# hpcaitech/SkyComputing

Measured on AMD Instinct MI355X. Metric: sec_per_iter_bert160_mnli_bsz32, lower is better.
Workload: dtype bf16; 1 GPU; model=bert-160L-H1024-A16, global_batch=32, seq_len=128, parallelism=pp1, microbatches=1, schedule=gpipe, allocate=even, num_pipeline_layers=483, hipgraph=True

## Files before the change

### skycomputing_amd/models/bert_layers.py

```python

from __future__ import annotations

import torch
import torch.nn as nn

from .. import ops
from ..registry import LAYER
from .bert import BertConfig


def _cfg(config) -> BertConfig:
    if isinstance(config, BertConfig):
        return config
    if isinstance(config, dict):
        return BertConfig.from_dict(config)
    raise TypeError(f"expected BertConfig or dict, got {type(config)}")


class SkyLayerNorm(nn.Module):

    def __init__(self, hidden_size: int, eps: float = 1e-12):
        super().__init__()
        self.weight = nn.Parameter(torch.ones(hidden_size))
        self.bias = nn.Parameter(torch.zeros(hidden_size))
# ... 107 lines not shown
    def activation_numel(self, batch: int, seq: int) -> int:
        return batch * seq * self.config.hidden_size + batch * seq


@LAYER.register_module(name="BertLayer_Head")
class BertLayerHead(nn.Module):

    def __init__(self, config):
        super().__init__()
        config = _cfg(config)
        self.config = config
        self.attention = BertSelfAttention(config)
        self.output = BertSelfOutput(config)

    def forward(self, hidden, ext_mask):
        attn = self.attention(hidden, ext_mask)
        out = self.output(attn, hidden)
        return out, ext_mask

    def layer_flops(self, batch: int, seq: int) -> float:
        H = self.config.hidden_size
        gemm = 4 * 2.0 * batch * seq * H * H
        attn = 2 * 2.0 * batch * self.config.num_attention_heads * seq * seq * (
            H // self.config.num_attention_heads
        )
        return gemm + attn

    def activation_numel(self, batch: int, seq: int) -> int:
        H = self.config.hidden_size
        h = self.config.num_attention_heads
        return 6 * batch * seq * H + 2 * batch * h * seq * seq

    def param_count(self) -> int:
# ... 106 lines not shown
```

### skycomputing_amd/ops/__init__.py

```python

from __future__ import annotations

import math
import os

import torch

from . import eager, hiplib
from .eager import ACT_FNS, gelu, swish

__all__ = [
    "layer_norm", "bias_gelu", "bias_tanh", "masked_softmax", "dropout",
    "attention_context", "linear_act", "linear_residual_layer_norm",
    "embedding_fused", "sgd_step",
    "gelu", "swish", "ACT_FNS", "hip_available",
]


def hip_available() -> bool:
    return hiplib.available()


def _use_hip(t: torch.Tensor) -> bool:
    if not t.is_cuda:
        return False
    if hiplib.available():
        return True
    if os.environ.get("SKY_ALLOW_EAGER_GPU") == "1":
# ... 107 lines not shown
        and _use_hip(x)
    ):
        from .functions import (
            LinearResidualLayerNormFn, ln_dbias_enabled, ln_xsum_width_ok,
        )

        if ln_dbias_enabled() and ln_xsum_width_ok(weight.shape[0]):
            p = dropout_p if training else 0.0
            return LinearResidualLayerNormFn.apply(
                x, weight, bias, ln_weight, ln_bias, eps, residual, p
            )
    return layer_norm(linear(x, weight, bias), ln_weight, ln_bias, eps,
                      residual, dropout_p, training)


def linear_act(x, weight, bias, act: str = "gelu"):
    if _use_hip(x) and act == "gelu" and bias is not None:
        from .functions import LinearGeluFn, _use_hblt

        if (_use_hblt() and os.environ.get("SKY_HBLT_GELU") == "1"
                and x.dtype == torch.float32 and weight.shape[0] % 8 == 0):
            return LinearGeluFn.apply(x, weight, bias)
        if x.dtype == torch.bfloat16:
            from .functions import _g2_enabled, _g2_fit

            rows = x.numel() // x.shape[-1]
            if (_g2_enabled("fwd", rows, weight.shape[0], weight.shape[1])
                    and _g2_fit(rows, weight.shape[0], weight.shape[1])):
                return LinearGeluFn.apply(x, weight, bias)
        y = torch.nn.functional.linear(x, weight)
# ... 25 lines not shown
```

### skycomputing_amd/ops/functions.py

```python

from __future__ import annotations

import os

import torch

from . import hiplib
from .hiplib import check, ptr

_DT = {torch.float32: 0, torch.bfloat16: 1}

_seed_gen = torch.Generator()
_seed_gen.manual_seed(0x5EED)


def set_dropout_seed(seed: int):
    _seed_gen.manual_seed(seed)


def _next_seed() -> int:
    return int(torch.randint(0, 2**62, (1,), generator=_seed_gen).item())


def _stream() -> int:
# ... 231 lines not shown
        "sky_masked_softmax_bwd",
    )
    dQ = torch.matmul(dS, k)
    dK = torch.matmul(dS.transpose(-1, -2), q)
    dqkv = torch.empty_like(qkv)
    check(
        lib.sky_pack3(
            _stream(), ptr(dQ.contiguous()), ptr(dK.contiguous()),
            ptr(dV.contiguous()), ptr(dqkv), B, S, h, d, _dt(qkv),
        ),
        "sky_pack3",
    )
    return dqkv


class FusedAttentionFn(torch.autograd.Function):

    @staticmethod
    def forward(ctx, qkv, mask, scale, dropout_p, training):
        lib = hiplib.require()
        B, S, three, h, d = qkv.shape
        assert three == 3 and d == 64 and S <= 128
        qkv = qkv.contiguous()
        mask = mask.contiguous() if mask is not None else None
        out = torch.empty(B, S, h, d, dtype=qkv.dtype, device=qkv.device)
        m = torch.empty(B, h, S, dtype=torch.float32, device=qkv.device)
        lsum = torch.empty_like(m)
        keep = 1.0 - dropout_p if (dropout_p > 0 and training) else 1.0
        salt = _next_seed() if keep < 1.0 else 0
        state = rng_state()
        check(
            lib.sky_attn_fwd(
                _stream(), ptr(qkv), ptr(mask), ptr(out), ptr(m), ptr(lsum),
                B, S, h, d, scale, keep, salt, state.data_ptr(),
            ),
            "sky_attn_fwd",
        )
        ctx.save_for_backward(qkv, mask, m, lsum)
        ctx.scale, ctx.keep, ctx.salt = scale, keep, salt
        return out

    @staticmethod
    def backward(ctx, dout):
        lib = hiplib.require()
        qkv, mask, m, lsum = ctx.saved_tensors
        B, S, _, h, d = qkv.shape
        dev = qkv.device
        if os.environ.get("SKY_NO_FUSED_ATTN_BWD") != "1":
            dout = dout.contiguous()
            dqkv = torch.empty_like(qkv)
            if os.environ.get("SKY_ATTN_FUSED_BWD") == "1":
                check(
                    lib.sky_attn_bwd_fused(
                        _stream(), ptr(qkv), ptr(dout), ptr(mask), ptr(m),
                        ptr(lsum), ptr(dqkv), B, S, h, d, ctx.scale,
                        ctx.keep, ctx.salt, rng_state().data_ptr(),
                    ),
                    "sky_attn_bwd_fused",
                )
                return dqkv, None, None, None, None
            alloc = torch.empty if S == 128 else torch.zeros
            n = B * h * S * S + (32 if S % 32 else 0)
            pdT = alloc(n, dtype=qkv.dtype, device=dev)
            dsT = alloc(n, dtype=qkv.dtype, device=dev)
            check(
                lib.sky_attn_bwd(
                    _stream(), ptr(qkv), ptr(dout), ptr(mask), ptr(m),
                    ptr(lsum), ptr(pdT), ptr(dsT), ptr(dqkv),
                    B, S, h, d, ctx.scale, ctx.keep, ctx.salt,
                    rng_state().data_ptr(),
                ),
                "sky_attn_bwd",
            )
            return dqkv, None, None, None, None
        P = torch.empty(B, h, S, S, dtype=qkv.dtype, device=dev)
        Pd = torch.empty_like(P) if ctx.keep < 1.0 else P
        check(
            lib.sky_attn_probs(
                _stream(), ptr(qkv), ptr(mask), ptr(m), ptr(lsum), ptr(P),
# ... 219 lines not shown


def gemm2_wgrad(dy2, x2):
    if dy2.dtype != torch.bfloat16:
        return None
    Kred, M = dy2.shape
    N = x2.shape[1]
    if not (_g2_enabled("wgrad", M, N, Kred) and _g2_fit(M, N, Kred)):
        return None
    dw = torch.empty(M, N, dtype=dy2.dtype, device=dy2.device)
    _g2_call(dy2, x2, dw, None, None, M, N, Kred, dy2.stride(0),
             x2.stride(0), dw.stride(0), 1, 1, 0, _g2_gsu(M, N, Kred))
    return dw


class LinearBiasFn(torch.autograd.Function):

    @staticmethod
    def forward(ctx, x, weight, bias):
        xs = x.shape
        x2 = x.reshape(-1, xs[-1])
        g2 = gemm2_fwd(x2 if x2.is_contiguous() else x2.contiguous(),
                       weight, bias)
        if g2 is not None:
            y = g2[0]
        else:
            y = torch.nn.functional.linear(x2, weight, bias)
        ctx.save_for_backward(x2, weight)
        ctx.xshape = xs
        ctx.has_bias = bias is not None
        return y.view(*xs[:-1], weight.shape[0])

    @staticmethod
    def backward(ctx, dy):
        x2, weight = ctx.saved_tensors
        dy2 = dy.reshape(-1, weight.shape[0])
        if not dy2.is_contiguous():
            dy2 = dy2.contiguous()
        dx = gemm2_dgrad(dy2, weight)
        dx = dx.view(ctx.xshape) if dx is not None else dy2.mm(weight).view(ctx.xshape)
        dw2 = gemm2_wgrad(dy2, x2 if x2.is_contiguous() else x2.contiguous())
        if dw2 is not None:
# ... 13 lines not shown
            )
            return dx, dw, db
        dw = dy2.t().mm(x2)
        db = colsum(dy2, weight.dtype) if ctx.has_bias else None
        return dx, dw, db


def ln_dbias_enabled() -> bool:
    return os.environ.get("SKY_NO_LN_DBIAS") != "1"


def ln_xsum_width_ok(cols: int) -> bool:
    return bool(hiplib.require().sky_layernorm_bwd_xsum_ok(cols))


class LinearResidualLayerNormFn(torch.autograd.Function):

    @staticmethod
    def forward(ctx, x, weight, bias, ln_w, ln_b, eps, residual, dropout_p=0.0):
        lib = hiplib.require()
        xs = x.shape
        x2 = x.reshape(-1, xs[-1])
        g2 = gemm2_fwd(x2 if x2.is_contiguous() else x2.contiguous(),
                       weight, bias)
        if g2 is not None:
            h = g2[0]
        else:
            h = torch.nn.functional.linear(x2, weight, bias)
        cols = weight.shape[0]
        h = h.view(*xs[:-1], cols).contiguous()
        residual = residual.contiguous() if residual is not None else None
        rows = h.numel() // cols
        y = torch.empty_like(h)
        mean = torch.empty(rows, dtype=torch.float32, device=h.device)
        rstd = torch.empty(rows, dtype=torch.float32, device=h.device)
        keep = 1.0 - dropout_p
        salt = _next_seed() if keep < 1.0 else 0
        state_ptr = rng_state().data_ptr() if keep < 1.0 else 0
        check(
            lib.sky_layernorm_fwd(
                _stream(), ptr(h), ptr(residual), ptr(ln_w), ptr(ln_b),
                ptr(y), ptr(mean), ptr(rstd), rows, cols, eps, _dt(h),
                keep, salt, state_ptr,
            ),
            "sky_layernorm_fwd",
        )
        ctx.save_for_backward(x2, weight, h, ln_w, mean, rstd)
        ctx.residual = residual
        ctx.has_residual = residual is not None
        ctx.keep, ctx.salt = keep, salt
        ctx.xshape = xs
        return y

    @staticmethod
    def backward(ctx, dy):
        lib = hiplib.require()
        x2, weight, h, ln_w, mean, rstd = ctx.saved_tensors
        dy = dy.contiguous()
        cols = h.shape[-1]
        rows = h.numel() // cols
        dh = torch.empty_like(h)
        d_ln_w = torch.empty(cols, dtype=ln_w.dtype, device=h.device)
        d_ln_b = torch.empty(cols, dtype=ln_w.dtype, device=h.device)
        dbias = torch.empty(cols, dtype=ln_w.dtype, device=h.device)
        scratch = _red_scratch(cols, 3, h.device)
        drop = ctx.keep < 1.0
        dres = torch.empty_like(h) if (drop and ctx.has_residual) else None
        state_ptr = rng_state().data_ptr() if drop else 0
        check(
            lib.sky_layernorm_bwd_xsum(
                _stream(), ptr(dy), ptr(h), ptr(ctx.residual), ptr(ln_w),
                ptr(mean), ptr(rstd), ptr(dh), ptr(d_ln_w), ptr(d_ln_b),
                ptr(scratch), rows, cols, _dt(h), ctx.keep, ctx.salt,
                state_ptr, ptr(dres), ptr(dbias),
            ),
            "sky_layernorm_bwd_xsum",
        )
        if not ctx.has_residual:
            dgrad_res = None
        elif drop:
            dgrad_res = dres
        else:
            dgrad_res = dh
        if dbias.dtype != weight.dtype:
            dbias = dbias.to(weight.dtype)
        dh2 = dh.view(-1, cols)
        dx = gemm2_dgrad(dh2, weight)
        dx = dx.view(ctx.xshape) if dx is not None else dh2.mm(weight).view(ctx.xshape)
        xc = x2 if x2.is_contiguous() else x2.contiguous()
        dw = gemm2_wgrad(dh2, xc)
        if dw is None and _use_hblt():
            M, K = xc.shape
            dw = torch.empty_like(weight)
            check(
                lib.sky_hblt_wgrad(
                    _stream(), ptr(xc), ptr(dh2), ptr(dw), M, cols, K, _dt(xc)
                ),
                "sky_hblt_wgrad",
            )
        elif dw is None:
            dw = dh2.t().mm(x2)
        return dx, dw, dbias, d_ln_w, d_ln_b, None, dgrad_res, None


class LinearGeluFn(torch.autograd.Function):

    @staticmethod
    def forward(ctx, x, weight, bias):
        xs = x.shape
        x2 = x.reshape(-1, xs[-1]).contiguous()
        M, K = x2.shape
        N = weight.shape[0]
        g2 = gemm2_fwd(x2, weight, bias, gelu=True, want_z=True)
        if g2 is not None:
            y, aux = g2
        else:
            lib = hiplib.require()
# ... 98 lines not shown
```

### skycomputing_amd/ops/hip/attention_bwd.hip

```cpp

#include "attn_common.h"

template <bool HAS_MASK>
__global__ __launch_bounds__(256, 3) void attn_bwd1s_kernel(
    const ushort_t* __restrict__ qkv, const ushort_t* __restrict__ dout,
    const ushort_t* __restrict__ mask, const float* __restrict__ m_io,
    const float* __restrict__ l_io, ushort_t* __restrict__ pdT,
    ushort_t* __restrict__ dsT, ushort_t* __restrict__ dqkv, int B, int S,
    int h, float scale, float keep, uint64_t salt,
    const unsigned long long* __restrict__ state) {
  extern __shared__ __attribute__((aligned(16))) char lds[];
  const int tid = threadIdx.x;
  const int l = tid & 63;
  const int w = tid >> 6;
  const int lm = l & 15;
  const int lg = l >> 4;
  const int QB = (S + 63) / 64;
  const int bh = blockIdx.x / QB;
  const int qb = blockIdx.x % QB;
  const int b = bh / h;
  const int hh = bh % h;
  const int ts = 3 * h * ATT_D;
  const int NT = (S + 15) / 16;
  const uint64_t seed = rng_seed(salt, state);
  const float inv_keep = 1.f / keep;
// ... 99 lines not shown
          *(ushort4_t*)(dsT + o) = ds4;
          *(ushort4_t*)(pdT + o) = pd4;
        } else {
#pragma unroll
          for (int r = 0; r < 4; ++r)
            if (qtok_base + lg * 4 + r < S) {
              dsT[o + r] = ds4[r];
              pdT[o + r] = pd4[r];
            }
        }
      }
    }
  }
  __syncthreads();

  if (active) {
    f32x4 qacc[4];
    att_zero(qacc);
#pragma unroll
    for (int ks = 0; ks < 4; ++ks) {
      if (ks * 32 >= S) break;
      bf16x8 asr = *(const bf16x8*)lds_at(
          lds, swz(32768 + w * 4096 + lm * 256 + (ks * 32 + lg * 8) * 2, lm, 15));
#pragma unroll
      for (int ct = 0; ct < 4; ++ct) {
        bf16x8 bkt = abf_tr_rows64(lds, 16384, ks * 32 + lg * 8, ct * 4, lm);
        qacc[ct] = __builtin_amdgcn_mfma_f32_16x16x32_bf16(asr, bkt, qacc[ct], 0, 0, 0);
      }
    }
    ushort_t* dq = dqkv + (size_t)b * S * ts + (size_t)hh * ATT_D;
    att_store_rows16(dq, ts, qacc, qtok_base, S, lm, lg);
  }
}

__global__ __launch_bounds__(256) void attn_bwd2_kernel(
    const ushort_t* __restrict__ qkv, const ushort_t* __restrict__ dout,
    const ushort_t* __restrict__ pdT, const ushort_t* __restrict__ dsT,
    ushort_t* __restrict__ dqkv, int B, int S, int h) {
  extern __shared__ __attribute__((aligned(16))) char lds[];
  const int tid = threadIdx.x;
  const int l = tid & 63;
  const int w = tid >> 6;
  const int lm = l & 15;
  const int lg = l >> 4;
  const int bh = blockIdx.x;
  const int b = bh / h;
  const int hh = bh % h;
  const int ts = 3 * h * ATT_D;
  const int dots = h * ATT_D;

  const ushort_t* qbase = qkv + (size_t)b * S * ts + (size_t)hh * ATT_D;
  const ushort_t* dobase = dout + ((size_t)b * S * h + hh) * ATT_D;

  att_glds_rows(qbase, ts, 0, S, false, S, lds, 0, tid);
  att_glds_rows(dobase, dots, 0, S, false, S, lds, 16384, tid);
  for (int u = S * 8 + tid; u < 128 * 8; u += 256) {
    *(ushort8_t*)lds_at(lds, 0 + u * 16) = (ushort8_t)(ushort_t)0;
    *(ushort8_t*)lds_at(lds, 16384 + u * 16) = (ushort8_t)(ushort_t)0;
  }
  asm volatile("s_waitcnt vmcnt(0)" ::: "memory");
  __syncthreads();

  const int kt0 = 2 * w;
  for (int ki = 0; ki < 2; ++ki) {
    const int ktok_base = (kt0 + ki) * 16;
    if (ktok_base >= S) break;
    int ktok = ktok_base + lm;
    if (ktok >= S) ktok = S - 1;
    f32x4 vacc[4], kacc[4];
    att_zero(vacc);
    att_zero(kacc);
#pragma unroll
    for (int ks = 0; ks < 4; ++ks) {
      if (ks * 32 >= S) break;
      const size_t abase = ((size_t)bh * S + ktok) * S + ks * 32 + lg * 8;
      bf16x8 apd = *(const bf16x8*)(pdT + abase);
      bf16x8 ads = *(const bf16x8*)(dsT + abase);
#pragma unroll
      for (int ct = 0; ct < 4; ++ct) {
        bf16x8 bdo = abf_tr_rows64(lds, 16384, ks * 32 + lg * 8, ct * 4, lm);
        vacc[ct] = __builtin_amdgcn_mfma_f32_16x16x32_bf16(apd, bdo, vacc[ct], 0, 0, 0);
        bf16x8 bq = abf_tr_rows64(lds, 0, ks * 32 + lg * 8, ct * 4, lm);
        kacc[ct] = __builtin_amdgcn_mfma_f32_16x16x32_bf16(ads, bq, kacc[ct], 0, 0, 0);
      }
    }
    ushort_t* dk = dqkv + (size_t)b * S * ts + (size_t)(h + hh) * ATT_D;
    ushort_t* dv = dqkv + (size_t)b * S * ts + (size_t)(2 * h + hh) * ATT_D;
    att_store_rows16x2(dk, dv, ts, kacc, vacc, ktok_base, S, lm, lg);
  }
}

#define ABF_K 0
#define ABF_Q (16 * 1024)
#define ABF_DO (32 * 1024)
#define ABF_DS (48 * 1024)
#define ABF_PD (64 * 1024)
#define ABF_LDS (80 * 1024)

template <bool HAS_MASK>
__global__ __launch_bounds__(256, 1) void attn_bwd_fused_kernel(
    const ushort_t* __restrict__ qkv, const ushort_t* __restrict__ dout,
    const ushort_t* __restrict__ mask, const float* __restrict__ m_io,
    const float* __restrict__ l_io, ushort_t* __restrict__ dqkv, int B,
// ... 177 lines not shown
                                  int64_t S, int64_t h, int64_t d,
                                  float scale, float keep, uint64_t salt,
                                  uint64_t state) {
  if (d != ATT_D || S > ATT_SMAX) return (int)hipErrorInvalidValue;
  hipStream_t s = (hipStream_t)stream;
  dim3 grid((unsigned)(B * h));
  ATT_LAUNCH_HM(mask != 0, (attn_bwd_fused_kernel<HM>), grid, ABF_LDS, s,
                (const ushort_t*)qkv, (const ushort_t*)dout,
                (const ushort_t*)mask, (const float*)m, (const float*)lsum,
                (ushort_t*)dqkv, (int)B, (int)S, (int)h, scale, keep, salt,
                (const unsigned long long*)state);
  LAUNCH_CHECK();
  return 0;
}

SKY_EXPORT int sky_attn_bwd(uint64_t stream, uint64_t qkv, uint64_t dout,
                            uint64_t mask, uint64_t m, uint64_t lsum,
                            uint64_t pdT, uint64_t dsT, uint64_t dqkv,
                            int64_t B, int64_t S, int64_t h, int64_t d,
                            float scale, float keep, uint64_t salt,
                            uint64_t state) {
  if (d != ATT_D || S > ATT_SMAX) return (int)hipErrorInvalidValue;
  hipStream_t s = (hipStream_t)stream;
  dim3 grid((unsigned)(B * h * ((S + 63) / 64)));
  ATT_LAUNCH_HM(mask != 0, (attn_bwd1s_kernel<HM>), grid, 48 * 1024, s,
                (const ushort_t*)qkv, (const ushort_t*)dout,
                (const ushort_t*)mask, (const float*)m, (const float*)lsum,
                (ushort_t*)pdT, (ushort_t*)dsT, (ushort_t*)dqkv, (int)B,
                (int)S, (int)h, scale, keep, salt,
                (const unsigned long long*)state);
  hipLaunchKernelGGL(attn_bwd2_kernel, dim3((unsigned)(B * h)), dim3(256),
                     32 * 1024, s, (const ushort_t*)qkv,
                     (const ushort_t*)dout, (const ushort_t*)pdT,
                     (const ushort_t*)dsT, (ushort_t*)dqkv, (int)B, (int)S,
                     (int)h);
  LAUNCH_CHECK();
  return 0;
}
```

### skycomputing_amd/ops/hip/attn_common.h

```cpp
#pragma once

#include "common.h"

typedef const __attribute__((address_space(1))) unsigned int* att_gas;
typedef __attribute__((address_space(3))) unsigned int* att_las;

typedef __attribute__((ext_vector_type(8))) short bf16x8;
typedef __attribute__((ext_vector_type(4))) float f32x4;

#define ATT_SMAX 128
#define ATT_D 64

DEV void* lds_at(char* base, int byte) { return (void*)(base + byte); }

DEV int swz(int byte_addr, int row, int rmask) {
  return byte_addr ^ ((row & rmask) << 4);
}

typedef __attribute__((ext_vector_type(4))) short s16x4_a;
typedef __attribute__((address_space(3))) s16x4_a* abf_las4;

DEV bf16x8 abf_tr_rows64(const char* lds_base, int off, int r0, int cq0,
                         int s4) {
  s16x4_a v[2];
// ... 121 lines not shown
                            int row0, int S, int lm, int lg) {
#pragma unroll
  for (int ct = 0; ct < 4; ++ct) {
#pragma unroll
    for (int r = 0; r < 4; ++r) {
      const int row = row0 + lg * 4 + r;
      const int c = ct * 16 + lm;
      if (row < S) {
        d0[(size_t)row * rstride + c] = f32_to_bf16(a0[ct][r]);
        d1[(size_t)row * rstride + c] = f32_to_bf16(a1[ct][r]);
      }
    }
  }
}

#define ATT_LAUNCH_HM(has_mask, KERNEL, grid, lds_bytes, stream, ...)         \
  do {                                                                        \
    if (has_mask) {                                                           \
      constexpr bool HM = true;                                               \
      hipLaunchKernelGGL(KERNEL, grid, dim3(256), lds_bytes, stream,          \
                         __VA_ARGS__);                                        \
    } else {                                                                  \
      constexpr bool HM = false;                                              \
      hipLaunchKernelGGL(KERNEL, grid, dim3(256), lds_bytes, stream,          \
                         __VA_ARGS__);                                        \
    }                                                                         \
  } while (0)
```

### skycomputing_amd/ops/hip/common.h

```cpp
#pragma once

#include <hip/hip_runtime.h>
#include <hip/hip_bf16.h>
#include <stdint.h>

#define WAVE 64
#define DEV __device__ __forceinline__

typedef unsigned short ushort_t;
typedef __attribute__((ext_vector_type(2))) unsigned short ushort2_t;
typedef __attribute__((ext_vector_type(4))) unsigned short ushort4_t;
typedef __attribute__((ext_vector_type(8))) unsigned short ushort8_t;
typedef __attribute__((ext_vector_type(4))) float float4_t;

DEV float bf16_to_f32(ushort_t u) {
  union { unsigned int i; float f; } v;
  v.i = ((unsigned int)u) << 16;
  return v.f;
}

DEV ushort_t f32_to_bf16(float f) {
  union { unsigned int i; float f; } v;
  v.f = f;
  unsigned int lsb = (v.i >> 16) & 1u;
// ... 108 lines not shown
  const float p = t * fmaf(t, fmaf(t, fmaf(t, fmaf(t, 1.061405429f, -1.453152027f),
                                           1.421413741f), -0.284496736f),
                           0.254829592f);
  const float r = 1.f - p * __expf(-ax * ax);
  return copysignf(r, x);
}
DEV float gelu_f(float x) { return 0.5f * x * (1.f + erf_fast(x * 0.70710678118654752f)); }
DEV float gelu_grad_f(float x) {
  const float k = 0.70710678118654752f;
  const float c = 0.3989422804014327f;
  float cdf = 0.5f * (1.f + erf_fast(x * k));
  float pdf = c * __expf(-0.5f * x * x);
  return cdf + x * pdf;
}

#define LAUNCH_CHECK() do { hipError_t e_ = hipGetLastError(); if (e_ != hipSuccess) return (int)e_; } while (0)

#define SKY_EXPORT extern "C" __attribute__((visibility("default")))
```

### skycomputing_amd/ops/hip/elementwise.hip

```cpp

#include "common.h"


template <int DT>
__global__ __launch_bounds__(256) void bias_gelu_fwd_vec_kernel(
    const void* __restrict__ x, const void* __restrict__ b,
    void* __restrict__ y, int64_t n8, int64_t cols8) {
  for (int64_t i8 = (int64_t)blockIdx.x * 256 + threadIdx.x; i8 < n8;
       i8 += (int64_t)gridDim.x * 256) {
    float v[8], bv[8];
    Vec8<DT>::load(x, i8, v);
    Vec8<DT>::load(b, i8 % cols8, bv);
#pragma unroll
    for (int j = 0; j < 8; ++j) v[j] = gelu_f(v[j] + bv[j]);
    Vec8<DT>::store(y, i8, v);
  }
}

template <int DT>
__global__ __launch_bounds__(256) void bias_gelu_fwd_kernel(
    const void* __restrict__ x, const void* __restrict__ b,
    void* __restrict__ y, int64_t n, int64_t cols) {
  for (int64_t i = (int64_t)blockIdx.x * 256 + threadIdx.x; i < n;
       i += (int64_t)gridDim.x * 256) {
// ... 153 lines not shown
  float s = 0.f;
  if (col < cols) {
    const int64_t y1 = min(nslabs, (int64_t)(g + 1) * per);
    for (int64_t y = (int64_t)g * per; y < y1; ++y)
      s += scratch[y * cols + col];
  }
  lds[g][c] = s;
  __syncthreads();
  for (int st = 32; st >= 1; st >>= 1) {
    if (g < st) lds[g][c] += lds[g + st][c];
    __syncthreads();
  }
  if (g == 0 && col < cols) store_elem<DTOUT>(out, col, lds[0][c]);
}

template <int DT, int BLOCK>
__global__ __launch_bounds__(BLOCK) void colsum_kernel(
    const void* __restrict__ src, float* __restrict__ out, int64_t rows,
    int64_t cols, int64_t rows_per_slab) {
  const int64_t col = (int64_t)blockIdx.x * BLOCK + threadIdx.x;
  if (col >= cols) return;
  const int64_t r0 = (int64_t)blockIdx.y * rows_per_slab;
  const int64_t r1 = min(rows, r0 + rows_per_slab);
  float s = 0.f;
  for (int64_t r = r0; r < r1; ++r) s += load_elem<DT>(src, r * cols + col);
  atomicAdd(&out[col], s);
}

template <int DT>
static void launch_colsum(hipStream_t s, const void* src, void* out,
                          float* scratch, int64_t rows, int64_t cols,
                          int dtout) {
  if (cols % 8 == 0 && scratch != nullptr) {
    constexpr int BLOCK = 128;
    const int64_t cols8 = cols / 8;
    const int64_t gx = (cols8 + BLOCK - 1) / BLOCK;
    int64_t nslabs = 1024 / gx;
    if (nslabs < 128) nslabs = 128;
    if (nslabs > CS_SLABS) nslabs = CS_SLABS;
    if (nslabs > rows) nslabs = rows;
    const int64_t slab = (rows + nslabs - 1) / nslabs;
    dim3 grid((unsigned)gx, (unsigned)nslabs);
    hipLaunchKernelGGL((colsum_part_kernel<DT, BLOCK>), grid, dim3(BLOCK), 0,
                       s, src, scratch, rows, cols8, slab);
    dim3 g2((unsigned)((cols + 15) / 16));
    if (dtout == DT_BF16)
      hipLaunchKernelGGL((colsum_final_kernel<256, DT_BF16>), g2, dim3(1024), 0,
                         s, scratch, out, cols, nslabs);
    else
      hipLaunchKernelGGL((colsum_final_kernel<256, DT_F32>), g2, dim3(1024), 0,
                         s, scratch, out, cols, nslabs);
    return;
  }
  constexpr int BLOCK = 256;
  int64_t slab = 64;
  while ((cols + BLOCK - 1) / BLOCK * ((rows + slab - 1) / slab) > 2048 && slab < rows)
    slab *= 2;
  dim3 grid((unsigned)((cols + BLOCK - 1) / BLOCK),
            (unsigned)((rows + slab - 1) / slab));
  (void)dtout;
  hipLaunchKernelGGL((colsum_kernel<DT, BLOCK>), grid, dim3(BLOCK), 0, s, src,
                     (float*)out, rows, cols, slab);
}

SKY_EXPORT int sky_colsum(uint64_t stream, uint64_t src, uint64_t out,
                          uint64_t scratch, int64_t rows, int64_t cols,
// ... 22 lines not shown
    if (nslabs > CS_SLABS) nslabs = CS_SLABS;
    if (nslabs > rows) nslabs = rows;
    const int64_t slab = (rows + nslabs - 1) / nslabs;
    dim3 grid((unsigned)(nwin * nslabs));
    auto launch_cs = [&](auto kern) {
      hipLaunchKernelGGL(kern, grid, dim3(256), 0, s, (const void*)dy,
                         (const void*)x, (const void*)b, (void*)dx,
                         (float*)scratch, rows, cols8, slab);
    };
    if (dt == DT_F32)
      hb ? launch_cs(bias_gelu_bwd_cs_kernel<DT_F32, true>)
         : launch_cs(bias_gelu_bwd_cs_kernel<DT_F32, false>);
    else
      hb ? launch_cs(bias_gelu_bwd_cs_kernel<DT_BF16, true>)
         : launch_cs(bias_gelu_bwd_cs_kernel<DT_BF16, false>);
    dim3 g2((unsigned)((cols + 15) / 16));
    if (dt == DT_BF16)
      hipLaunchKernelGGL((colsum_final_kernel<256, DT_BF16>), g2, dim3(1024),
                         0, s, (float*)scratch, (void*)db, cols, nslabs);
    else
      hipLaunchKernelGGL((colsum_final_kernel<256, DT_F32>), g2, dim3(1024),
                         0, s, (float*)scratch, (void*)db, cols, nslabs);
    LAUNCH_CHECK();
    return 0;
  }
  if (cols % 8 == 0 && scratch != 0 && getenv("SKY_GELU_FUSED_BWD")) {
    constexpr int BLOCK = 128;
    const int64_t cols8 = cols / 8;
    const int64_t gx = (cols8 + BLOCK - 1) / BLOCK;
    int64_t nslabs = 4096 / gx;
    if (nslabs < 128) nslabs = 128;
    if (nslabs > CS_SLABS) nslabs = CS_SLABS;
    if (nslabs > rows) nslabs = rows;
    const int64_t slab = (rows + nslabs - 1) / nslabs;
    dim3 grid((unsigned)gx, (unsigned)nslabs);
    auto launch_part = [&](auto kern) {
      hipLaunchKernelGGL(kern, grid, dim3(BLOCK), 0, s, (const void*)dy,
                         (const void*)x, (const void*)b, (void*)dx,
                         (float*)scratch, rows, cols8, slab);
    };
    if (dt == DT_F32)
      hb ? launch_part(bias_gelu_bwd_part_kernel<DT_F32, true, BLOCK>)
         : launch_part(bias_gelu_bwd_part_kernel<DT_F32, false, BLOCK>);
    else
      hb ? launch_part(bias_gelu_bwd_part_kernel<DT_BF16, true, BLOCK>)
         : launch_part(bias_gelu_bwd_part_kernel<DT_BF16, false, BLOCK>);
    dim3 g2((unsigned)((cols + 15) / 16));
    if (dt == DT_BF16)
      hipLaunchKernelGGL((colsum_final_kernel<256, DT_BF16>), g2, dim3(1024),
                         0, s, (float*)scratch, (void*)db, cols, nslabs);
    else
      hipLaunchKernelGGL((colsum_final_kernel<256, DT_F32>), g2, dim3(1024),
                         0, s, (float*)scratch, (void*)db, cols, nslabs);
    LAUNCH_CHECK();
    return 0;
  }
  if (cols % 8 == 0) {
    int64_t n8 = n / 8;
    unsigned grid = (unsigned)((n8 + 255) / 256);
    if (grid > 2048u) grid = 2048u;
    auto launch_vec = [&](auto kern) {
      hipLaunchKernelGGL(kern, dim3(grid), dim3(256), 0, s, (const void*)dy,
                         (const void*)x, (const void*)b, (void*)dx, n8, cols / 8);
    };
    if (dt == DT_F32)
      hb ? launch_vec(bias_gelu_bwd_dx_vec_kernel<DT_F32, true>)
         : launch_vec(bias_gelu_bwd_dx_vec_kernel<DT_F32, false>);
    else
// ... 112 lines not shown
```

### skycomputing_amd/ops/hiplib.py

```python

from __future__ import annotations

import ctypes
import os

_LIB = None
_LIB_PATH = os.path.join(os.path.dirname(os.path.abspath(__file__)), "hip", "libskyhip.so")
_TRIED = False

_SIGNATURES: dict[str, list] = {}

u64 = ctypes.c_uint64
i64 = ctypes.c_int64
i32 = ctypes.c_int32
f32 = ctypes.c_float
f64 = ctypes.c_double


def _register_signatures(lib):
    sigs = {
        "sky_layernorm_fwd": [u64, u64, u64, u64, u64, u64, u64, u64, i64, i64, f32, i32, f32, u64, u64],
        "sky_layernorm_bwd": [u64, u64, u64, u64, u64, u64, u64, u64, u64, u64, u64, i64, i64, i32, f32, u64, u64, u64],
        "sky_layernorm_bwd_xsum": [u64, u64, u64, u64, u64, u64, u64, u64, u64, u64, u64, i64, i64, i32, f32, u64, u64, u64, u64],
        "sky_layernorm_bwd_xsum_ok": [i64],
# ... 9 lines not shown
        "sky_dropout_bwd": [u64, u64, u64, i64, f32, u64, u64, i32],
        "sky_rng_tick": [u64, u64],
        "sky_colsum": [u64, u64, u64, u64, i64, i64, i32, i32],
        "sky_hblt_wgrad_bgrad": [u64, u64, u64, u64, u64, i64, i64, i64, i32],
        "sky_hblt_wgrad": [u64, u64, u64, u64, i64, i64, i64, i32],
        "sky_hblt_linear_gelu_aux": [u64, u64, u64, u64, u64, u64, i64, i64, i64, i32, i32],
        "sky_mfma_probe": [u64, u64, u64, u64],
        "sky_glds_probe": [u64, u64, u64, i32],
        "sky_gemm": [u64, u64, u64, u64, u64, u64, i64, i64, i64, i64, i64, i64, i32, i32, i32, i32, i32],
        "sky_gemm2": [u64, u64, u64, u64, u64, u64, u64, i64, i64, i64, i64, i64, i64, i32, i32, i32, i32],
        "sky_pack3": [u64, u64, u64, u64, u64, i64, i64, i64, i64, i32],
        "sky_attn_fwd": [u64, u64, u64, u64, u64, u64, i64, i64, i64, i64, f32, f32, u64, u64],
        "sky_attn_probs": [u64, u64, u64, u64, u64, u64, u64, i64, i64, i64, i64, f32, f32, u64, u64],
        "sky_attn_flash_fwd": [u64, u64, u64, u64, u64, u64, i64, i64, i64, i64, f32, f32, u64, u64],
        "sky_attn_bwd": [u64] * 9 + [i64, i64, i64, i64, f32, f32, u64, u64],
        "sky_attn_bwd_fused": [u64] * 7 + [i64, i64, i64, i64, f32, f32, u64, u64],
    }
    for name, argtypes in sigs.items():
        if hasattr(lib, name):
            fn = getattr(lib, name)
            fn.argtypes = argtypes
            fn.restype = ctypes.c_int
    return sigs


def lib():
    global _LIB, _TRIED
    if _LIB is None and not _TRIED:
        _TRIED = True
        if os.path.isfile(_LIB_PATH):
# ... 29 lines not shown
```

Before: 0.1059 sec/iter.

## Fuse attention head block and compute QKV bias grad inside attention backward

New measurement: 0.1033 sec/iter, median of 6. 1.03x faster.

```diff
diff --git a/skycomputing_amd/models/bert_layers.py b/skycomputing_amd/models/bert_layers.py
--- a/skycomputing_amd/models/bert_layers.py
+++ b/skycomputing_amd/models/bert_layers.py
@@ -145,9 +145,13 @@
         self.output = BertSelfOutput(config)
 
     def forward(self, hidden, ext_mask):
-        attn = self.attention(hidden, ext_mask)
-        out = self.output(attn, hidden)
-        return out, ext_mask
+        att, out = self.attention, self.output
+        y = ops.attention_block(
+            hidden, ext_mask, att.qkv.weight, att.qkv.bias, att.num_heads,
+            att.dropout_p, out.dense.weight, out.dense.bias,
+            out.layer_norm.weight, out.layer_norm.bias, out.layer_norm.eps,
+            out.dropout_p, self.training)
+        return y, ext_mask
 
     def layer_flops(self, batch: int, seq: int) -> float:
         H = self.config.hidden_size
diff --git a/skycomputing_amd/ops/__init__.py b/skycomputing_amd/ops/__init__.py
--- a/skycomputing_amd/ops/__init__.py
+++ b/skycomputing_amd/ops/__init__.py
@@ -11,7 +11,8 @@
 
 __all__ = [
     "layer_norm", "bias_gelu", "bias_tanh", "masked_softmax", "dropout",
-    "attention_context", "linear_act", "linear_residual_layer_norm",
+    "attention_context", "attention_block", "linear_act",
+    "linear_residual_layer_norm",
     "embedding_fused", "sgd_step",
     "gelu", "swish", "ACT_FNS", "hip_available",
 ]
@@ -149,6 +150,39 @@
                       residual, dropout_p, training)
 
 
+def attention_block(hidden, mask, qkv_weight, qkv_bias, num_heads: int,
+                    attn_dropout_p: float, out_weight, out_bias, ln_weight,
+                    ln_bias, eps: float = 1e-12, hidden_dropout_p: float = 0.0,
+                    training: bool = False):
+    B, S, H = hidden.shape
+    d = H // num_heads
+    if (
+        hidden.is_cuda and hidden.dtype == torch.bfloat16 and d == 64
+        and S <= 128 and qkv_bias is not None and out_bias is not None
+        and hiplib.available()
+        and os.environ.get("SKY_NO_FUSED_ATTN") != "1"
+        and os.environ.get("SKY_NO_FUSED_ATTN_BWD") != "1"
+        and os.environ.get("SKY_ATTN_FUSED_BWD") != "1"
+    ):
+        from .functions import (
+            AttentionBlockFn, attn_block_enabled, ln_dbias_enabled,
+            ln_xsum_width_ok,
+        )
+
+        if attn_block_enabled() and ln_dbias_enabled() and ln_xsum_width_ok(H):
+            ap = attn_dropout_p if (training and attn_dropout_p > 0) else 0.0
+            hp = hidden_dropout_p if training else 0.0
+            return AttentionBlockFn.apply(
+                hidden, qkv_weight, qkv_bias, mask, num_heads, ap,
+                out_weight, out_bias, ln_weight, ln_bias, eps, hp
+            )
+    qkv = linear(hidden, qkv_weight, qkv_bias).view(B, S, 3, num_heads, d)
+    attn = attention(qkv, mask, attn_dropout_p, training)
+    return linear_residual_layer_norm(
+        attn, out_weight, out_bias, ln_weight, ln_bias, eps, hidden,
+        hidden_dropout_p, training)
+
+
 def linear_act(x, weight, bias, act: str = "gelu"):
     if _use_hip(x) and act == "gelu" and bias is not None:
         from .functions import LinearGeluFn, _use_hblt
diff --git a/skycomputing_amd/ops/functions.py b/skycomputing_amd/ops/functions.py
--- a/skycomputing_amd/ops/functions.py
+++ b/skycomputing_amd/ops/functions.py
@@ -1,6 +1,7 @@
 
 from __future__ import annotations
 
+import math
 import os
 
 import torch
@@ -269,28 +270,42 @@
     return dqkv
 
 
+def _attn_fwd(qkv, mask, scale, keep):
+    lib = hiplib.require()
+    B, S, _, h, d = qkv.shape
+    out = torch.empty(B, S, h, d, dtype=qkv.dtype, device=qkv.device)
+    m = torch.empty(B, h, S, dtype=torch.float32, device=qkv.device)
+    lsum = torch.empty_like(m)
+    salt = _next_seed() if keep < 1.0 else 0
+    state = rng_state()
+    check(
+        lib.sky_attn_fwd(
+            _stream(), ptr(qkv), ptr(mask), ptr(out), ptr(m), ptr(lsum),
+            B, S, h, d, scale, keep, salt, state.data_ptr(),
+        ),
+        "sky_attn_fwd",
+    )
+    return out, m, lsum, salt
+
+
+def _attn_bwd_scratch(qkv):
+    B, S, _, h, _ = qkv.shape
+    alloc = torch.empty if S == 128 else torch.zeros
+    n = B * h * S * S + (32 if S % 32 else 0)
+    return (alloc(n, dtype=qkv.dtype, device=qkv.device),
+            alloc(n, dtype=qkv.dtype, device=qkv.device))
+
+
 class FusedAttentionFn(torch.autograd.Function):
 
     @staticmethod
     def forward(ctx, qkv, mask, scale, dropout_p, training):
-        lib = hiplib.require()
         B, S, three, h, d = qkv.shape
         assert three == 3 and d == 64 and S <= 128
         qkv = qkv.contiguous()
         mask = mask.contiguous() if mask is not None else None
-        out = torch.empty(B, S, h, d, dtype=qkv.dtype, device=qkv.device)
-        m = torch.empty(B, h, S, dtype=torch.float32, device=qkv.device)
-        lsum = torch.empty_like(m)
         keep = 1.0 - dropout_p if (dropout_p > 0 and training) else 1.0
-        salt = _next_seed() if keep < 1.0 else 0
-        state = rng_state()
-        check(
-            lib.sky_attn_fwd(
-                _stream(), ptr(qkv), ptr(mask), ptr(out), ptr(m), ptr(lsum),
-                B, S, h, d, scale, keep, salt, state.data_ptr(),
-            ),
-            "sky_attn_fwd",
-        )
+        out, m, lsum, salt = _attn_fwd(qkv, mask, scale, keep)
         ctx.save_for_backward(qkv, mask, m, lsum)
         ctx.scale, ctx.keep, ctx.salt = scale, keep, salt
         return out
@@ -314,10 +329,7 @@
                     "sky_attn_bwd_fused",
                 )
                 return dqkv, None, None, None, None
-            alloc = torch.empty if S == 128 else torch.zeros
-            n = B * h * S * S + (32 if S % 32 else 0)
-            pdT = alloc(n, dtype=qkv.dtype, device=dev)
-            dsT = alloc(n, dtype=qkv.dtype, device=dev)
+            pdT, dsT = _attn_bwd_scratch(qkv)
             check(
                 lib.sky_attn_bwd(
                     _stream(), ptr(qkv), ptr(dout), ptr(mask), ptr(m),
@@ -567,18 +579,43 @@
     return dw
 
 
+def _linear_fwd(x2, weight, bias):
+    g2 = gemm2_fwd(x2 if x2.is_contiguous() else x2.contiguous(), weight, bias)
+    if g2 is not None:
+        return g2[0]
+    return torch.nn.functional.linear(x2, weight, bias)
+
+
+def _wgrad_plain(dy2, x2, weight):
+    xc = x2 if x2.is_contiguous() else x2.contiguous()
+    dw = gemm2_wgrad(dy2, xc)
+    if dw is None and _use_hblt():
+        M, K = xc.shape
+        dw = torch.empty_like(weight)
+        check(
+            hiplib.require().sky_hblt_wgrad(
+                _stream(), ptr(xc), ptr(dy2), ptr(dw), M, weight.shape[0], K,
+                _dt(xc)
+            ),
+            "sky_hblt_wgrad",
+        )
+    elif dw is None:
+        dw = dy2.t().mm(x2)
+    return dw
+
+
+def _dgrad(dy2, weight):
+    dx = gemm2_dgrad(dy2, weight)
+    return dx if dx is not None else dy2.mm(weight)
+
+
 class LinearBiasFn(torch.autograd.Function):
 
     @staticmethod
     def forward(ctx, x, weight, bias):
         xs = x.shape
         x2 = x.reshape(-1, xs[-1])
-        g2 = gemm2_fwd(x2 if x2.is_contiguous() else x2.contiguous(),
-                       weight, bias)
-        if g2 is not None:
-            y = g2[0]
-        else:
-            y = torch.nn.functional.linear(x2, weight, bias)
+        y = _linear_fwd(x2, weight, bias)
         ctx.save_for_backward(x2, weight)
         ctx.xshape = xs
         ctx.has_bias = bias is not None
@@ -622,37 +659,61 @@
     return bool(hiplib.require().sky_layernorm_bwd_xsum_ok(cols))
 
 
+def _ln_fwd(h, residual, ln_w, ln_b, eps, keep):
+    cols = h.shape[-1]
+    rows = h.numel() // cols
+    y = torch.empty_like(h)
+    mean = torch.empty(rows, dtype=torch.float32, device=h.device)
+    rstd = torch.empty(rows, dtype=torch.float32, device=h.device)
+    salt = _next_seed() if keep < 1.0 else 0
+    state_ptr = rng_state().data_ptr() if keep < 1.0 else 0
+    check(
+        hiplib.require().sky_layernorm_fwd(
+            _stream(), ptr(h), ptr(residual), ptr(ln_w), ptr(ln_b),
+            ptr(y), ptr(mean), ptr(rstd), rows, cols, eps, _dt(h),
+            keep, salt, state_ptr,
+        ),
+        "sky_layernorm_fwd",
+    )
+    return y, mean, rstd, salt
+
+
+def _ln_bwd_xsum(dy, h, residual, ln_w, mean, rstd, keep, salt):
+    cols = h.shape[-1]
+    rows = h.numel() // cols
+    dh = torch.empty_like(h)
+    d_ln_w = torch.empty(cols, dtype=ln_w.dtype, device=h.device)
+    d_ln_b = torch.empty(cols, dtype=ln_w.dtype, device=h.device)
+    dxsum = torch.empty(cols, dtype=ln_w.dtype, device=h.device)
+    scratch = _red_scratch(cols, 3, h.device)
+    drop = keep < 1.0
+    dres = torch.empty_like(h) if (drop and residual is not None) else None
+    state_ptr = rng_state().data_ptr() if drop else 0
+    check(
+        hiplib.require().sky_layernorm_bwd_xsum(
+            _stream(), ptr(dy), ptr(h), ptr(residual), ptr(ln_w),
+            ptr(mean), ptr(rstd), ptr(dh), ptr(d_ln_w), ptr(d_ln_b),
+            ptr(scratch), rows, cols, _dt(h), keep, salt,
+            state_ptr, ptr(dres), ptr(dxsum),
+        ),
+        "sky_layernorm_bwd_xsum",
+    )
+    if residual is not None and not drop:
+        dres = dh
+    return dh, d_ln_w, d_ln_b, dxsum, dres
+
+
 class LinearResidualLayerNormFn(torch.autograd.Function):
 
     @staticmethod
     def forward(ctx, x, weight, bias, ln_w, ln_b, eps, residual, dropout_p=0.0):
-        lib = hiplib.require()
         xs = x.shape
         x2 = x.reshape(-1, xs[-1])
-        g2 = gemm2_fwd(x2 if x2.is_contiguous() else x2.contiguous(),
-                       weight, bias)
-        if g2 is not None:
-            h = g2[0]
-        else:
-            h = torch.nn.functional.linear(x2, weight, bias)
         cols = weight.shape[0]
-        h = h.view(*xs[:-1], cols).contiguous()
+        h = _linear_fwd(x2, weight, bias).view(*xs[:-1], cols).contiguous()
         residual = residual.contiguous() if residual is not None else None
-        rows = h.numel() // cols
-        y = torch.empty_like(h)
-        mean = torch.empty(rows, dtype=torch.float32, device=h.device)
-        rstd = torch.empty(rows, dtype=torch.float32, device=h.device)
         keep = 1.0 - dropout_p
-        salt = _next_seed() if keep < 1.0 else 0
-        state_ptr = rng_state().data_ptr() if keep < 1.0 else 0
-        check(
-            lib.sky_layernorm_fwd(
-                _stream(), ptr(h), ptr(residual), ptr(ln_w), ptr(ln_b),
-                ptr(y), ptr(mean), ptr(rstd), rows, cols, eps, _dt(h),
-                keep, salt, state_ptr,
-            ),
-            "sky_layernorm_fwd",
-        )
+        y, mean, rstd, salt = _ln_fwd(h, residual, ln_w, ln_b, eps, keep)
         ctx.save_for_backward(x2, weight, h, ln_w, mean, rstd)
         ctx.residual = residual
         ctx.has_residual = residual is not None
@@ -662,53 +723,85 @@
 
     @staticmethod
     def backward(ctx, dy):
-        lib = hiplib.require()
         x2, weight, h, ln_w, mean, rstd = ctx.saved_tensors
-        dy = dy.contiguous()
-        cols = h.shape[-1]
-        rows = h.numel() // cols
-        dh = torch.empty_like(h)
-        d_ln_w = torch.empty(cols, dtype=ln_w.dtype, device=h.device)
-        d_ln_b = torch.empty(cols, dtype=ln_w.dtype, device=h.device)
-        dbias = torch.empty(cols, dtype=ln_w.dtype, device=h.device)
-        scratch = _red_scratch(cols, 3, h.device)
-        drop = ctx.keep < 1.0
-        dres = torch.empty_like(h) if (drop and ctx.has_residual) else None
-        state_ptr = rng_state().data_ptr() if drop else 0
-        check(
-            lib.sky_layernorm_bwd_xsum(
-                _stream(), ptr(dy), ptr(h), ptr(ctx.residual), ptr(ln_w),
-                ptr(mean), ptr(rstd), ptr(dh), ptr(d_ln_w), ptr(d_ln_b),
-                ptr(scratch), rows, cols, _dt(h), ctx.keep, ctx.salt,
-                state_ptr, ptr(dres), ptr(dbias),
-            ),
-            "sky_layernorm_bwd_xsum",
-        )
-        if not ctx.has_residual:
-            dgrad_res = None
-        elif drop:
-            dgrad_res = dres
-        else:
-            dgrad_res = dh
+        dh, d_ln_w, d_ln_b, dbias, dgrad_res = _ln_bwd_xsum(
+            dy.contiguous(), h, ctx.residual, ln_w, mean, rstd, ctx.keep,
+            ctx.salt)
         if dbias.dtype != weight.dtype:
             dbias = dbias.to(weight.dtype)
-        dh2 = dh.view(-1, cols)
-        dx = gemm2_dgrad(dh2, weight)
-        dx = dx.view(ctx.xshape) if dx is not None else dh2.mm(weight).view(ctx.xshape)
-        xc = x2 if x2.is_contiguous() else x2.contiguous()
-        dw = gemm2_wgrad(dh2, xc)
-        if dw is None and _use_hblt():
-            M, K = xc.shape
-            dw = torch.empty_like(weight)
-            check(
-                lib.sky_hblt_wgrad(
-                    _stream(), ptr(xc), ptr(dh2), ptr(dw), M, cols, K, _dt(xc)
-                ),
-                "sky_hblt_wgrad",
-            )
-        elif dw is None:
-            dw = dh2.t().mm(x2)
+        dh2 = dh.view(-1, h.shape[-1])
+        dx = _dgrad(dh2, weight).view(ctx.xshape)
+        dw = _wgrad_plain(dh2, x2, weight)
         return dx, dw, dbias, d_ln_w, d_ln_b, None, dgrad_res, None
+
+
+def attn_block_enabled() -> bool:
+    return os.environ.get("SKY_NO_ATTN_BLOCK") != "1"
+
+
+class AttentionBlockFn(torch.autograd.Function):
+
+    @staticmethod
+    def forward(ctx, hidden, wqkv, bqkv, mask, num_heads, attn_p, wo, bo,
+                ln_w, ln_b, eps, hidden_p):
+        B, S, H = hidden.shape
+        d = H // num_heads
+        assert d == 64 and S <= 128 and hidden.dtype == torch.bfloat16
+        hidden = hidden.contiguous()
+        x2 = hidden.view(-1, H)
+        qkv = _linear_fwd(x2, wqkv, bqkv).view(B, S, 3, num_heads, d)
+        mask = mask.contiguous() if mask is not None else None
+        scale = 1.0 / math.sqrt(d)
+        akeep = 1.0 - attn_p
+        ctxl, m, lsum, asalt = _attn_fwd(qkv, mask, scale, akeep)
+        c2 = ctxl.view(-1, H)
+        h = _linear_fwd(c2, wo, bo).view(B, S, H)
+        keep = 1.0 - hidden_p
+        y, mean, rstd, salt = _ln_fwd(h, hidden, ln_w, ln_b, eps, keep)
+        ctx.save_for_backward(x2, wqkv, qkv, mask, m, lsum, c2, wo, h, ln_w,
+                              mean, rstd)
+        ctx.scale, ctx.akeep, ctx.asalt = scale, akeep, asalt
+        ctx.keep, ctx.salt = keep, salt
+        return y
+
+    @staticmethod
+    def backward(ctx, dy):
+        lib = hiplib.require()
+        (x2, wqkv, qkv, mask, m, lsum, c2, wo, h, ln_w, mean,
+         rstd) = ctx.saved_tensors
+        B, S, _, nh, d = qkv.shape
+        H = nh * d
+        dh, d_ln_w, d_ln_b, dbo, dres = _ln_bwd_xsum(
+            dy.contiguous(), h, x2, ln_w, mean, rstd, ctx.keep, ctx.salt)
+        dh2 = dh.view(-1, H)
+        dctx = _dgrad(dh2, wo)
+        dwo = _wgrad_plain(dh2, c2, wo)
+        dqkv = torch.empty_like(qkv)
+        dbqkv = torch.empty(3 * H, dtype=wqkv.dtype, device=qkv.device)
+        pdT, dsT = _attn_bwd_scratch(qkv)
+        slabs = torch.empty(B * ((S + 63) // 64) * 3 * H, dtype=torch.float32,
+                            device=qkv.device)
+        check(
+            lib.sky_attn_bwd_dbias(
+                _stream(), ptr(qkv), ptr(dctx), ptr(mask), ptr(m), ptr(lsum),
+                ptr(pdT), ptr(dsT), ptr(dqkv), B, S, nh, d, ctx.scale,
+                ctx.akeep, ctx.asalt, rng_state().data_ptr(), ptr(slabs),
+                ptr(dbqkv), _dt(dbqkv),
+            ),
+            "sky_attn_bwd_dbias",
+        )
+        dqkv2 = dqkv.view(-1, 3 * H)
+        dwqkv = _wgrad_plain(dqkv2, x2, wqkv)
+        dres2 = dres.view(-1, H)
+        g2 = gemm2_dgrad(dqkv2, wqkv)
+        if g2 is not None:
+            dres2.add_(g2)
+        else:
+            dres2.addmm_(dqkv2, wqkv)
+        if dbo.dtype != wo.dtype:
+            dbo = dbo.to(wo.dtype)
+        return (dres.view(B, S, H), dwqkv, dbqkv, None, None, None, dwo, dbo,
+                d_ln_w, d_ln_b, None, None)
 
 
 class LinearGeluFn(torch.autograd.Function):
diff --git a/skycomputing_amd/ops/hip/attention_bwd.hip b/skycomputing_amd/ops/hip/attention_bwd.hip
--- a/skycomputing_amd/ops/hip/attention_bwd.hip
+++ b/skycomputing_amd/ops/hip/attention_bwd.hip
@@ -1,14 +1,14 @@
 
 #include "attn_common.h"
 
-template <bool HAS_MASK>
+template <bool HAS_MASK, bool DBIAS>
 __global__ __launch_bounds__(256, 3) void attn_bwd1s_kernel(
     const ushort_t* __restrict__ qkv, const ushort_t* __restrict__ dout,
     const ushort_t* __restrict__ mask, const float* __restrict__ m_io,
     const float* __restrict__ l_io, ushort_t* __restrict__ pdT,
     ushort_t* __restrict__ dsT, ushort_t* __restrict__ dqkv, int B, int S,
     int h, float scale, float keep, uint64_t salt,
-    const unsigned long long* __restrict__ state) {
+    const unsigned long long* __restrict__ state, float* __restrict__ dbscr) {
   extern __shared__ __attribute__((aligned(16))) char lds[];
   const int tid = threadIdx.x;
   const int l = tid & 63;
@@ -138,6 +138,7 @@
   }
   __syncthreads();
 
+  float cs[4] = {0.f, 0.f, 0.f, 0.f};
   if (active) {
     f32x4 qacc[4];
     att_zero(qacc);
@@ -154,13 +155,28 @@
     }
     ushort_t* dq = dqkv + (size_t)b * S * ts + (size_t)hh * ATT_D;
     att_store_rows16(dq, ts, qacc, qtok_base, S, lm, lg);
-  }
-}
-
+    if constexpr (DBIAS) att_colsum_rows16(cs, qacc, qtok_base, S, lg);
+  }
+  if constexpr (DBIAS) {
+    float* wsum = (float*)lds_at(lds, 0);
+    att_colsum_wave(cs);
+    if (lg == 0) {
+#pragma unroll
+      for (int ct = 0; ct < 4; ++ct) wsum[w * 64 + ct * 16 + lm] = cs[ct];
+    }
+    __syncthreads();
+    if (tid < 64)
+      dbscr[((size_t)b * QB + qb) * ts + (size_t)hh * ATT_D + tid] =
+          (wsum[tid] + wsum[64 + tid]) + (wsum[128 + tid] + wsum[192 + tid]);
+  }
+}
+
+template <bool DBIAS>
 __global__ __launch_bounds__(256) void attn_bwd2_kernel(
     const ushort_t* __restrict__ qkv, const ushort_t* __restrict__ dout,
     const ushort_t* __restrict__ pdT, const ushort_t* __restrict__ dsT,
-    ushort_t* __restrict__ dqkv, int B, int S, int h) {
+    ushort_t* __restrict__ dqkv, int B, int S, int h,
+    float* __restrict__ dbscr) {
   extern __shared__ __attribute__((aligned(16))) char lds[];
   const int tid = threadIdx.x;
   const int l = tid & 63;
@@ -186,6 +202,7 @@
   __syncthreads();
 
   const int kt0 = 2 * w;
+  float ck[4] = {0.f, 0.f, 0.f, 0.f}, cv[4] = {0.f, 0.f, 0.f, 0.f};
   for (int ki = 0; ki < 2; ++ki) {
     const int ktok_base = (kt0 + ki) * 16;
     if (ktok_base >= S) break;
@@ -211,6 +228,30 @@
     ushort_t* dk = dqkv + (size_t)b * S * ts + (size_t)(h + hh) * ATT_D;
     ushort_t* dv = dqkv + (size_t)b * S * ts + (size_t)(2 * h + hh) * ATT_D;
     att_store_rows16x2(dk, dv, ts, kacc, vacc, ktok_base, S, lm, lg);
+    if constexpr (DBIAS) {
+      att_colsum_rows16(ck, kacc, ktok_base, S, lg);
+      att_colsum_rows16(cv, vacc, ktok_base, S, lg);
+    }
+  }
+  if constexpr (DBIAS) {
+    float* wsum = (float*)lds_at(lds, 32768);
+    att_colsum_wave(ck);
+    att_colsum_wave(cv);
+    if (lg == 0) {
+#pragma unroll
+      for (int ct = 0; ct < 4; ++ct) {
+        wsum[w * 128 + ct * 16 + lm] = ck[ct];
+        wsum[w * 128 + 64 + ct * 16 + lm] = cv[ct];
+      }
+    }
+    __syncthreads();
+    if (tid < 128) {
+      const int QB = (S + 63) / 64;
+      const size_t col = (size_t)((tid < 64 ? h : 2 * h) + hh) * ATT_D + (tid & 63);
+      float* dst = dbscr + (size_t)b * QB * ts + col;
+      dst[0] = (wsum[tid] + wsum[128 + tid]) + (wsum[256 + tid] + wsum[384 + tid]);
+      for (int q = 1; q < QB; ++q) dst[(size_t)q * ts] = 0.f;
+    }
   }
 }
 
@@ -418,6 +459,27 @@
   return 0;
 }
 
+template <bool DBIAS>
+static void launch_attn_bwd_pair(hipStream_t s, uint64_t qkv, uint64_t dout,
+                                 uint64_t mask, uint64_t m, uint64_t lsum,
+                                 uint64_t pdT, uint64_t dsT, uint64_t dqkv,
+                                 int64_t B, int64_t S, int64_t h, float scale,
+                                 float keep, uint64_t salt, uint64_t state,
+                                 float* dbscr) {
+  dim3 grid((unsigned)(B * h * ((S + 63) / 64)));
+  ATT_LAUNCH_HM(mask != 0, (attn_bwd1s_kernel<HM, DBIAS>), grid, 48 * 1024, s,
+                (const ushort_t*)qkv, (const ushort_t*)dout,
+                (const ushort_t*)mask, (const float*)m, (const float*)lsum,
+                (ushort_t*)pdT, (ushort_t*)dsT, (ushort_t*)dqkv, (int)B,
+                (int)S, (int)h, scale, keep, salt,
+                (const unsigned long long*)state, dbscr);
+  hipLaunchKernelGGL(attn_bwd2_kernel<DBIAS>, dim3((unsigned)(B * h)),
+                     dim3(256), (DBIAS ? 34 : 32) * 1024, s,
+                     (const ushort_t*)qkv, (const ushort_t*)dout,
+                     (const ushort_t*)pdT, (const ushort_t*)dsT,
+                     (ushort_t*)dqkv, (int)B, (int)S, (int)h, dbscr);
+}
+
 SKY_EXPORT int sky_attn_bwd(uint64_t stream, uint64_t qkv, uint64_t dout,
                             uint64_t mask, uint64_t m, uint64_t lsum,
                             uint64_t pdT, uint64_t dsT, uint64_t dqkv,
@@ -425,19 +487,27 @@
                             float scale, float keep, uint64_t salt,
                             uint64_t state) {
   if (d != ATT_D || S > ATT_SMAX) return (int)hipErrorInvalidValue;
-  hipStream_t s = (hipStream_t)stream;
-  dim3 grid((unsigned)(B * h * ((S + 63) / 64)));
-  ATT_LAUNCH_HM(mask != 0, (attn_bwd1s_kernel<HM>), grid, 48 * 1024, s,
-                (const ushort_t*)qkv, (const ushort_t*)dout,
-                (const ushort_t*)mask, (const float*)m, (const float*)lsum,
-                (ushort_t*)pdT, (ushort_t*)dsT, (ushort_t*)dqkv, (int)B,
-                (int)S, (int)h, scale, keep, salt,
-                (const unsigned long long*)state);
-  hipLaunchKernelGGL(attn_bwd2_kernel, dim3((unsigned)(B * h)), dim3(256),
-                     32 * 1024, s, (const ushort_t*)qkv,
-                     (const ushort_t*)dout, (const ushort_t*)pdT,
-                     (const ushort_t*)dsT, (ushort_t*)dqkv, (int)B, (int)S,
-                     (int)h);
+  launch_attn_bwd_pair<false>((hipStream_t)stream, qkv, dout, mask, m, lsum,
+                              pdT, dsT, dqkv, B, S, h, scale, keep, salt,
+                              state, nullptr);
   LAUNCH_CHECK();
   return 0;
 }
+
+SKY_EXPORT int sky_attn_bwd_dbias(uint64_t stream, uint64_t qkv, uint64_t dout,
+                                  uint64_t mask, uint64_t m, uint64_t lsum,
+                                  uint64_t pdT, uint64_t dsT, uint64_t dqkv,
+                                  int64_t B, int64_t S, int64_t h, int64_t d,
+                                  float scale, float keep, uint64_t salt,
+                                  uint64_t state, uint64_t scratch,
+                                  uint64_t dbias, int dbias_dt) {
+  if (d != ATT_D || S > ATT_SMAX || scratch == 0 || dbias == 0)
+    return (int)hipErrorInvalidValue;
+  hipStream_t s = (hipStream_t)stream;
+  launch_attn_bwd_pair<true>(s, qkv, dout, mask, m, lsum, pdT, dsT, dqkv, B, S,
+                             h, scale, keep, salt, state, (float*)scratch);
+  sky_launch_colsum_final(s, (const float*)scratch, (void*)dbias,
+                          3 * h * ATT_D, B * ((S + 63) / 64), dbias_dt);
+  LAUNCH_CHECK();
+  return 0;
+}
diff --git a/skycomputing_amd/ops/hip/attn_common.h b/skycomputing_amd/ops/hip/attn_common.h
--- a/skycomputing_amd/ops/hip/attn_common.h
+++ b/skycomputing_amd/ops/hip/attn_common.h
@@ -159,6 +159,24 @@
   }
 }
 
+DEV void att_colsum_rows16(float (&cs)[4], const f32x4 (&acc)[4], int row0,
+                           int S, int lg) {
+#pragma unroll
+  for (int ct = 0; ct < 4; ++ct) {
+#pragma unroll
+    for (int r = 0; r < 4; ++r)
+      if (row0 + lg * 4 + r < S) cs[ct] += bf16_to_f32(f32_to_bf16(acc[ct][r]));
+  }
+}
+
+DEV void att_colsum_wave(float (&cs)[4]) {
+#pragma unroll
+  for (int ct = 0; ct < 4; ++ct) {
+    cs[ct] += __shfl_xor(cs[ct], 16, 64);
+    cs[ct] += __shfl_xor(cs[ct], 32, 64);
+  }
+}
+
 #define ATT_LAUNCH_HM(has_mask, KERNEL, grid, lds_bytes, stream, ...)         \
   do {                                                                        \
     if (has_mask) {                                                           \
diff --git a/skycomputing_amd/ops/hip/common.h b/skycomputing_amd/ops/hip/common.h
--- a/skycomputing_amd/ops/hip/common.h
+++ b/skycomputing_amd/ops/hip/common.h
@@ -146,6 +146,9 @@
   return cdf + x * pdf;
 }
 
+void sky_launch_colsum_final(hipStream_t s, const float* scratch, void* out,
+                             int64_t cols, int64_t nslabs, int dtout);
+
 #define LAUNCH_CHECK() do { hipError_t e_ = hipGetLastError(); if (e_ != hipSuccess) return (int)e_; } while (0)
 
 #define SKY_EXPORT extern "C" __attribute__((visibility("default")))
diff --git a/skycomputing_amd/ops/hip/elementwise.hip b/skycomputing_amd/ops/hip/elementwise.hip
--- a/skycomputing_amd/ops/hip/elementwise.hip
+++ b/skycomputing_amd/ops/hip/elementwise.hip
@@ -191,6 +191,17 @@
   if (g == 0 && col < cols) store_elem<DTOUT>(out, col, lds[0][c]);
 }
 
+void sky_launch_colsum_final(hipStream_t s, const float* scratch, void* out,
+                             int64_t cols, int64_t nslabs, int dtout) {
+  dim3 g2((unsigned)((cols + 15) / 16));
+  if (dtout == DT_BF16)
+    hipLaunchKernelGGL((colsum_final_kernel<256, DT_BF16>), g2, dim3(1024), 0,
+                       s, scratch, out, cols, nslabs);
+  else
+    hipLaunchKernelGGL((colsum_final_kernel<256, DT_F32>), g2, dim3(1024), 0,
+                       s, scratch, out, cols, nslabs);
+}
+
 template <int DT, int BLOCK>
 __global__ __launch_bounds__(BLOCK) void colsum_kernel(
     const void* __restrict__ src, float* __restrict__ out, int64_t rows,
@@ -220,13 +231,7 @@
     dim3 grid((unsigned)gx, (unsigned)nslabs);
     hipLaunchKernelGGL((colsum_part_kernel<DT, BLOCK>), grid, dim3(BLOCK), 0,
                        s, src, scratch, rows, cols8, slab);
-    dim3 g2((unsigned)((cols + 15) / 16));
-    if (dtout == DT_BF16)
-      hipLaunchKernelGGL((colsum_final_kernel<256, DT_BF16>), g2, dim3(1024), 0,
-                         s, scratch, out, cols, nslabs);
-    else
-      hipLaunchKernelGGL((colsum_final_kernel<256, DT_F32>), g2, dim3(1024), 0,
-                         s, scratch, out, cols, nslabs);
+    sky_launch_colsum_final(s, scratch, out, cols, nslabs, dtout);
     return;
   }
   constexpr int BLOCK = 256;
@@ -279,13 +284,7 @@
     else
       hb ? launch_cs(bias_gelu_bwd_cs_kernel<DT_BF16, true>)
          : launch_cs(bias_gelu_bwd_cs_kernel<DT_BF16, false>);
-    dim3 g2((unsigned)((cols + 15) / 16));
-    if (dt == DT_BF16)
-      hipLaunchKernelGGL((colsum_final_kernel<256, DT_BF16>), g2, dim3(1024),
-                         0, s, (float*)scratch, (void*)db, cols, nslabs);
-    else
-      hipLaunchKernelGGL((colsum_final_kernel<256, DT_F32>), g2, dim3(1024),
-                         0, s, (float*)scratch, (void*)db, cols, nslabs);
+    sky_launch_colsum_final(s, (const float*)scratch, (void*)db, cols, nslabs, dt);
     LAUNCH_CHECK();
     return 0;
   }
@@ -310,13 +309,7 @@
     else
       hb ? launch_part(bias_gelu_bwd_part_kernel<DT_BF16, true, BLOCK>)
          : launch_part(bias_gelu_bwd_part_kernel<DT_BF16, false, BLOCK>);
-    dim3 g2((unsigned)((cols + 15) / 16));
-    if (dt == DT_BF16)
-      hipLaunchKernelGGL((colsum_final_kernel<256, DT_BF16>), g2, dim3(1024),
-                         0, s, (float*)scratch, (void*)db, cols, nslabs);
-    else
-      hipLaunchKernelGGL((colsum_final_kernel<256, DT_F32>), g2, dim3(1024),
-                         0, s, (float*)scratch, (void*)db, cols, nslabs);
+    sky_launch_colsum_final(s, (const float*)scratch, (void*)db, cols, nslabs, dt);
     LAUNCH_CHECK();
     return 0;
   }
diff --git a/skycomputing_amd/ops/hiplib.py b/skycomputing_amd/ops/hiplib.py
--- a/skycomputing_amd/ops/hiplib.py
+++ b/skycomputing_amd/ops/hiplib.py
@@ -47,6 +47,7 @@
         "sky_attn_probs": [u64, u64, u64, u64, u64, u64, u64, i64, i64, i64, i64, f32, f32, u64, u64],
         "sky_attn_flash_fwd": [u64, u64, u64, u64, u64, u64, i64, i64, i64, i64, f32, f32, u64, u64],
         "sky_attn_bwd": [u64] * 9 + [i64, i64, i64, i64, f32, f32, u64, u64],
+        "sky_attn_bwd_dbias": [u64] * 9 + [i64, i64, i64, i64, f32, f32, u64, u64, u64, u64, i32],
         "sky_attn_bwd_fused": [u64] * 7 + [i64, i64, i64, i64, f32, f32, u64, u64],
     }
     for name, argtypes in sigs.items():
```
